# Fr4nz83/kubernetes-scheduler-simulator

Measured on AMD Instinct MI355X. Metric: pods scheduled/sec + node-score evals/sec (FGD, openb trace) at 1/2/4/8 MI355X, higher is better.
Workload: dtype int32+f64

## Files before the change

kubernetes-scheduler-simulator_amd/csrc/ksim_memo.hpp:

```cpp
#pragma once

namespace ksim_memo {

using namespace ksim;
using namespace ksim_plan::memo;

constexpr int kMBlock = 1024;
constexpr int kMWaves = kMBlock / 64;
constexpr int kMaxItems = 1 + 8 * kMaxCw;
constexpr int kCritWaves = 9;
constexpr unsigned kScanMask = 0x7C00u;
constexpr int kScanWaves = __builtin_popcount(kScanMask);
static_assert((kScanMask & ((2u << kCritWaves) - 1u)) == 0u && (kScanMask >> (kMWaves - 1)) == 0u,
              "the scan waves are idle in phase A on an owner too");
constexpr int kEvBuf = 128;
constexpr unsigned kSpinLimit = 1u << 22;
constexpr int kMaxDeadWords = 32;
constexpr int kLag = 3;
constexpr int kTopN = kLag + 1;
constexpr int kTopWords = 8;
constexpr int kDItems = kLag * 9;

struct MemoArgs {
  ReplicaDev* reps;
  const int* rep_list;
  const int* wg_map;
  int N, K, Cw;
  int nfw;
  int Cmax;
  const PodDev* cls_pod;
  const int* cls_owner;
  const int* wg_cls;
  const int* wg_ref;
  const unsigned long long* wg_grp;
  const int* ev_owner;
  const double* th;
  unsigned* win;
  int win_stride;
  int* fail;
  unsigned long long* prof;
  unsigned long long* trace;
  int trace_steps;
  int decider;
  const int* ev_cls;
  unsigned* topg;
  int skip;
  int delay;
  unsigned* hkeys;
  int* started;
  int gate_epoch;
};
constexpr int kTrace = 4;
constexpr int kProfPhases = 24;

struct __align__(16) MemoShared {
  PodDev ev[kEvBuf];
  int evo[kEvBuf + 8];
  unsigned dead[kMaxDeadWords];
  PodDev cls[kMaxCw];
  TypDev tp[kMaxTypical];
  NodeRec dnode;
  unsigned dfirst;
  unsigned pad_dfirst[3];
  double th[104];
  unsigned long long grp[kMaxCw];
  int cls_id[kMaxCw];
  int sc_ref[kMaxCw];
  int cnt[kMaxCw];
  unsigned ikey[kMaxItems + 3];
  double F[kMaxItems + 1];
  double Fc[10];
  uint8_t item_code[kMaxItems + 7];
  uint8_t item_slot[kMaxItems + 7];
  unsigned wtop[kMWaves][2];
  unsigned wtop4[kMWaves][kTopN];
  unsigned t2a, t2b;
  int nitems;
  int crit_done;
  int dirty;
  int stop;
  unsigned pay;
  unsigned long long prof[kProfPhases];
};
static_assert(sizeof(MemoShared) % 16 == 0, "keep the node records 16-B aligned");
static_assert(sizeof(MemoShared) == kSharedBytes, "memo_layout (ksim_plan.hpp) starts the node records after MemoShared");

KSIM_HD unsigned pack_key32(int score, int rank, int gf) {
  return ((unsigned)(score + 1) << 24) | ((unsigned)(kMemoMaxRank - rank) << 12) | ((unsigned)gf << 8);
}
KSIM_HD int key32_score(unsigned k) { return (int)(k >> 24) - 1; }
KSIM_HD int key32_rank(unsigned k) { return kMemoMaxRank - (int)((k >> 12) & 0xFFFu); }
KSIM_HD int key32_gpu(unsigned k) {
  const int gf = (int)((k >> 8) & 0xFu);
  return gf ? 15 - gf : -1;
}

KSIM_HD unsigned pack_pay(int rank, int mask) {
  return 1u | ((unsigned)(rank + 1) << 8) | ((unsigned)(mask & 0xff) << 24);
}

template <typename T>
__device__ __forceinline__ void gput(T* p, const T& v) {
  static_assert(sizeof(T) % 4 == 0, "word-sized records");
  const unsigned* src = reinterpret_cast<const unsigned*>(&v);
  __attribute__((address_space(1))) unsigned* dst = (__attribute__((address_space(1))) unsigned*)(p);
#pragma unroll
  for (int i = 0; i < (int)(sizeof(T) / 4); ++i) dst[i] = src[i];
}
template <typename T>
__device__ __forceinline__ T gget(const T* p) {
  static_assert(sizeof(T) % 4 == 0, "word-sized records");
  T v;
  unsigned* dst = reinterpret_cast<unsigned*>(&v);
  const __attribute__((address_space(1))) unsigned* src = (const __attribute__((address_space(1))) unsigned*)(p);
#pragma unroll
  for (int i = 0; i < (int)(sizeof(T) / 4); ++i) dst[i] = src[i];
  return v;
}
__device__ __forceinline__ void gput_node(NodeRec* p, const NodeV& n) {
  uint4* q = reinterpret_cast<uint4*>(p);
  gput(q, make_uint4((uint32_t)n.cpu_left, (uint32_t)n.mem_left, n.g[0], n.g[1]));
  gput(q + 1, make_uint4(n.g[2], n.g[3], n.meta, n.name_rank));
}

__device__ __forceinline__ unsigned gload32(const unsigned* p) {
  return __hip_atomic_load(p, __ATOMIC_RELAXED, __HIP_MEMORY_SCOPE_AGENT);
}
__device__ __forceinline__ void gstore32(unsigned* p, unsigned v) {
  __hip_atomic_store(p, v, __ATOMIC_RELAXED, __HIP_MEMORY_SCOPE_AGENT);
}
__device__ __forceinline__ double readlane_d(double v, int l) {
  const unsigned long long u = __builtin_bit_cast(unsigned long long, v);
  const unsigned lo = (unsigned)__builtin_amdgcn_readlane((int)(unsigned)u, l);
  const unsigned hi = (unsigned)__builtin_amdgcn_readlane((int)(unsigned)(u >> 32), l);
  return __builtin_bit_cast(double, ((unsigned long long)hi << 32) | lo);
}

__device__ __forceinline__ unsigned ge_mask(const NodeV& n, int m) {
  using ksim_replay::u16x2;
  const uint32_t mp = (uint32_t)m * 0x10001u;
  unsigned lt = 0u;
#pragma unroll
  for (int i = 0; i < 4; ++i) {
    const u16x2 d = (u16x2)(__builtin_bit_cast(u16x2, n.g[i]) - __builtin_bit_cast(u16x2, mp)) >> (u16x2){15, 15};
    const uint32_t x = __builtin_bit_cast(uint32_t, d);
    lt |= ((x & 1u) | ((x >> 15) & 2u)) << (2 * i);
  }
  return ~lt & 0xFFu;
}

__device__ __forceinline__ int score_lookup_dev(double delta, const double* th) {
  const float e = __builtin_amdgcn_exp2f((float)delta * -0.0014426950408889634f);
  int a = (int)(100.0f * __builtin_amdgcn_rcpf(1.0f + e));
  a = a < 0 ? 0 : (a > 100 ? 100 : a);
  if (delta >= th[a + 1]) ++a;
  else if (delta < th[a]) --a;
  return a;
}

__device__ __forceinline__ unsigned first_mask_lanes(const NodeV& n, int lane) {
  const int g = lane & 7;
  const int v = ksim_replay::gl_dyn(n, g);
  const bool first = lane < 8 && g < n.gpu_cnt() && (ksim_replay::gl_equal_mask(n, v) & ((1u << g) - 1u)) == 0u;
  return (unsigned)__ballot(first) & 0xFFu;
}

__device__ __forceinline__ void merge2(unsigned& a1, unsigned& a2, unsigned b1, unsigned b2) {
// ... 372 lines not shown
        if (lane == 0) s_last[rk] = step;
      }
      if (rk >= 0 && lane == 0) store_node(&ds.hprev[step % kLag], before);
      const unsigned fa = rk >= 0 ? first_mask_lanes(after, lane) : 0u;
      hn2 = hn1; ha2 = ha1; hf2 = hf1;
      hn1 = hn0; ha1 = ha0; hf1 = hf0;
      hn0 = rk; ha0 = after; hf0 = fa;
      dmark(23);
    }
    if (lane == 0) lds_store(&ds.finished, 1);
  } else if (wv == kPW) {
    int chunk = 0, my_cls = -1;
    for (int step = 0; step < E; ++step) {
      if (step == 0 || step - chunk >= 64) {
        chunk = step;
        my_cls = step + lane < E ? gget(a.ev_cls + gbase + step + lane) : -1;
      }
      if (__builtin_amdgcn_readlane(my_cls, step - chunk) < 0) continue;
      unsigned cspins = 0;
      while (lds_load(&ds.consumed) < step - kRing) {
        if (lds_load(&sh.stop) || lds_load(&ds.finished) || !lds_spin(cspins, &sh.stop, a.fail)) break;
      }
      if (lds_load(&sh.stop) || lds_load(&ds.finished)) break;
      unsigned v = 0u;
      bool ok = true;
      if (lane <= kTopN) {
        const unsigned* tw = a.topg + (gbase + step) * kTopWords;
        unsigned spins = 0;
        while ((v = gload32(tw + lane)) == 0u) {
          if (++spins > kSpinLimit || lds_load(&sh.stop)) { ok = false; break; }
          __builtin_amdgcn_s_sleep(1);
        }
      }
      if (__ballot(!ok) != 0ull) {
        if (lane == 0) { lds_store(&sh.stop, 1); atomicOr(a.fail, 1); }
        break;
      }
      const int slot = step % kRing;
      if (lane <= kTopN) ds.ring[slot][lane] = v;
      lds_release();
      if (lane == 0) lds_store(&ds.ring_tag[slot], step + 1);
    }
  } else if (wv <= nF) {
    int seen = 0;
    for (;;) {
      int cf;
      unsigned spins = 0;
      while ((cf = lds_load(&ds.cflag)) == seen) {
        if (lds_load(&ds.finished) || lds_load(&sh.stop) || !lds_spin(spins, &sh.stop, a.fail)) break;
        __builtin_amdgcn_s_sleep(2);
      }
      if (cf == seen) break;
      seen = cf;
      lds_acquire();
      const int nit = __builtin_amdgcn_readfirstlane(ds.nitems);
      const PodDev cp = ksim_replay::uniform_pod(&ds.cp);
      for (int it = wv - 1; it < nit; it += nF) {
        const NodeV cur = ksim_replay::uniform_node(&ds.xcur[ds.item_x[it]]);
        int cpuL, total;
        uint32_t gs[4];
        ksim_replay::fgd_candidate(cur, ds.item_code[it], cp, &cpuL, gs, &total);
        const double F = wave_F(cpuL, gs, total, 1u << cur.gpu_type(), rp.typed != 0, sh.tp, rp.ncpu, rp.nt, lane,
                                s_fold + (size_t)wv * kFoldBuf);
        if (lane == 0) ds.F[it] = F;
      }
      lds_release();
      if (lane == 0) __hip_atomic_fetch_add(&ds.fdone, 1, __ATOMIC_RELAXED, __HIP_MEMORY_SCOPE_WORKGROUP);
    }
  }
  __syncthreads();
}

template <bool kDecider, bool kGeneral, bool kStress = false, bool kReport = false, bool kHKeys = false>
__global__ __launch_bounds__(kMBlock) void k_memo(MemoArgs a, const TypDev* __restrict__ tp_all) {
  static_assert(!(kDecider && kHKeys), "the decider's scratch aliases the LDS keys");
  constexpr bool kDelays = kGeneral || kStress;
  extern __shared__ __attribute__((aligned(16))) char smem[];
  MemoShared& sh = *reinterpret_cast<MemoShared*>(smem);
  constexpr int kLW = kMWaves - 1;
  const int gw = a.wg_map[blockIdx.x];
  const int gi = gw >> 8;
  const int r = a.rep_list[gi];
  const int w = gw & 0xff;
  const int tid = (int)threadIdx.x, lane = tid & 63, wv = tid >> 6;
  const ReplicaDev rp = a.reps[r];
  const TypDev* __restrict__ tp = tp_all + (size_t)r * kMaxTypical;
  const int N = a.N, Cw = a.Cw;
  const int* rank2idx = reinterpret_cast<const int*>(rp.tags + (size_t)N * kTagStride);
  NodeRec* s_nodes = reinterpret_cast<NodeRec*>(smem + sizeof(MemoShared));
  unsigned* s_keys = kHKeys ? a.hkeys + (size_t)blockIdx.x * Cw * N : reinterpret_cast<unsigned*>(s_nodes + N);
  double* s_fold = reinterpret_cast<double*>(
      reinterpret_cast<char*>(s_nodes + N) + (kHKeys ? 0 : (std::max((size_t)Cw * N * 4, sizeof(DeciderScratch)) + 15) & ~(size_t)15));
  int* s_last = reinterpret_cast<int*>(reinterpret_cast<char*>(s_fold) +
                                       std::max((size_t)a.nfw * kFoldBuf * 8, ((size_t)N * 8 + 15) & ~(size_t)15));
  const PodDev* cls_pod = a.cls_pod + (size_t)gi * a.Cmax;
  const size_t wgo = (size_t)blockIdx.x * Cw;
  unsigned* win = a.win + (size_t)gi * a.win_stride;
  const int* evo = a.ev_owner + (size_t)gi * a.win_stride;
  const bool is_w0 = w == 0;
  constexpr bool kSkip = !kDecider && !kGeneral;
  const bool skip_ok = kSkip && a.skip && a.Cmax <= kMaxDeadWords * 32;

  for (int i = tid; i < N; i += kMBlock) {
    store_node(&s_nodes[i], load_node(rp.nodes + rank2idx[i]));
    s_last[i] = -1;
  }
  for (int j = tid; j < kMaxCw; j += kMBlock) {
    const int cid = j < Cw ? a.wg_cls[wgo + j] : -1;
    sh.cls_id[j] = cid;
    sh.sc_ref[j] = j < Cw ? a.wg_ref[wgo + j] : j;
    sh.grp[j] = j < Cw ? a.wg_grp[wgo + j] : 0ull;
    sh.cnt[j] = 0;
    if (cid >= 0) sh.cls[j] = cls_pod[cid];
    else reinterpret_cast<uint4*>(&sh.cls[j])[0] = reinterpret_cast<uint4*>(&sh.cls[j])[1] = make_uint4(0, 0, 0, 0);
  }
  for (int i = tid; i < rp.nt * 2; i += kMBlock)
    reinterpret_cast<uint4*>(sh.tp)[i] = reinterpret_cast<const uint4*>(tp)[i];
  if (tid == 0) { sh.dirty = -1; sh.stop = 0; sh.nitems = 0; sh.t2a = 0u; sh.t2b = 0u; sh.pay = 0u; sh.crit_done = 0; }
  if (a.started != nullptr && tid == 0)
    __hip_atomic_store(a.started + blockIdx.x, a.gate_epoch, __ATOMIC_RELAXED, __HIP_MEMORY_SCOPE_SYSTEM);
  for (int i = tid; i < kMaxDeadWords; i += kMBlock) sh.dead[i] = 0u;
  const bool prof = kGeneral && a.prof != nullptr;
  unsigned long long* const trace = kGeneral ? a.trace : nullptr;
  if (prof && tid < kProfPhases) sh.prof[tid] = 0ull;
  unsigned long long t_last = prof ? __builtin_amdgcn_s_memrealtime() : 0ull;
  const unsigned long long t_start = t_last, c_start = prof ? __builtin_amdgcn_s_memtime() : 0ull;
  auto mark = [&](int ph) {
    if (prof && tid == 0) {
      const unsigned long long t = __builtin_amdgcn_s_memrealtime();
      sh.prof[ph] += t - t_last;
      t_last = t;
    }
  };
  __syncthreads();
  double* s_F0 = s_fold;
  for (int i = tid; i < N; i += kMBlock) s_F0[i] = eval_fgd_item(load_node(&s_nodes[i]), 0, PodDev{}, rp, tp);
  __syncthreads();
  for (int x = tid; x < Cw * N; x += kMBlock) {
    const int j = x / N, i = x - j * N;
    unsigned k = 0u;
    if (sh.cls_id[j] >= 0) k = memo_key_scalar(load_node(&s_nodes[i]), sh.cls[j], s_F0[i], i, rp, tp);
    s_keys[x] = k;
  }
  __syncthreads();
  for (int i = tid; i < a.nfw * kFoldBuf; i += kMBlock) s_fold[i] = 0.0;
  for (int j = wv; j < Cw; j += kMWaves) {
    int c = 0;
    for (int i0 = 0; i0 < N; i0 += 64) c += __popcll(__ballot(i0 + lane < N && s_keys[(size_t)j * N + i0 + lane] != 0u));
    if (lane == 0) sh.cnt[j] = c;
  }

  auto top2 = [&](int slot) {
    const unsigned* kr = s_keys + (size_t)slot * N;
    unsigned a1 = 0u, a2 = 0u;
    for (int i = tid; i < N; i += kMBlock) {
      const unsigned k = kr[i];
      if (k > a1) { a2 = a1; a1 = k; } else if (k > a2) { a2 = k; }
    }
    wave_top2(a1, a2);
    if (lane == 0) { sh.wtop[wv][0] = a1; sh.wtop[wv][1] = a2; }
    __syncthreads();
    if (wv == 0) {
      a1 = lane < kMWaves ? sh.wtop[lane][0] : 0u;
      a2 = lane < kMWaves ? sh.wtop[lane][1] : 0u;
      wave_top2(a1, a2);
      if (lane == 0) { sh.t2a = a1; sh.t2b = a2; }
    }
  };
  const bool use_th = !kGeneral || a.th != nullptr;
  if (use_th)
    for (int i = tid; i < 102; i += kMBlock) sh.th[i] = a.th[i];
  const size_t gbase = (size_t)gi * a.win_stride;
  auto publish_top = [&](int slot, int sp) {
    const unsigned* kr = s_keys + (size_t)slot * N;
    unsigned k4[4];
#pragma unroll
    for (int q = 0; q < 4; ++q) k4[q] = tid + q * kMBlock < N ? kr[tid + q * kMBlock] : 0u;
    unsigned prev = 0xFFFFFFFFu;
#pragma unroll
    for (int r = 0; r < kTopN; ++r) {
      unsigned c = 0u;
#pragma unroll
      for (int q = 0; q < 4; ++q) c = (k4[q] < prev && k4[q] > c) ? k4[q] : c;
      const unsigned m = (unsigned)ksim_replay::wave_max_dpp((int)c);
      if (lane == 0) sh.wtop4[wv][r] = m;
      prev = m;
    }
    __syncthreads();
    if (wv == 0) {
      const unsigned v = lane < kMWaves * kTopN ? sh.wtop4[lane / kTopN][lane % kTopN] : 0u;
      unsigned pv = 0xFFFFFFFFu, out = 0u;
#pragma unroll
      for (int r = 0; r < kTopN; ++r) {
        const unsigned m = (unsigned)ksim_replay::wave_max_dpp((int)(v < pv ? v : 0u));
        out = lane == r ? m : out;
        pv = m;
      }
      unsigned* tw = a.topg + (gbase + sp) * kTopWords;
      if (lane < kTopN) gstore32(tw + lane, out | 1u);
      else if (lane == kTopN) gstore32(tw + lane, ((unsigned)sh.cnt[slot] << 8) | 1u);
    }
  };
  if constexpr (kDecider) {
    for (int sp = 0; sp < kLag && sp < rp.n_events; ++sp) {
      const int o = evo[sp];
      __syncthreads();
      if (o >= 0 && (o >> 16) == w) publish_top(o & 0xff, sp);
    }
  } else {
    int s0 = 0;
    while (s0 < rp.n_events && evo[s0] < 0) ++s0;
    __syncthreads();
    if (s0 < rp.n_events && (evo[s0] >> 16) == w) top2(evo[s0] & 0xff);
  }
  __syncthreads();
  mark(0);
  auto score_of = [&](double delta) { return use_th ? score_lookup_dev(delta, sh.th) : fgd_score_of_delta(delta); };

  PodDev lq{};
  bool l_valid = false, l_rep = false, l_share = false;
  int l_ref = 0;
  unsigned long long l_grp = 0ull;
  if (wv == kLW) {
    l_valid = lane < Cw && sh.cls_id[lane] >= 0;
    if (l_valid) lq = sh.cls[lane];
    l_ref = sh.sc_ref[lane];
    l_grp = sh.grp[lane];
    l_rep = l_valid && l_ref == lane;
    l_share = is_share_pod(lq);
  }
  bool r_feas = false, r_need = false, r_skip = false;
  int r_base = 0, r_ni = 0;

  const bool decider = kDecider && w == 0;
  if constexpr (kDecider)
    if (decider) memo_decider(a, rp, sh, s_nodes, *reinterpret_cast<DeciderScratch*>(s_keys), s_fold, s_last, gi, tid);
  for (int step = 0; step < (decider ? 0 : rp.n_events); ++step) {
    const int eb = step & (kEvBuf - 1);
    if (eb == 0) {
      const int ne = min(kEvBuf, rp.n_events - step);
      const uint4* src = reinterpret_cast<const uint4*>(rp.ev + step);
      for (int i = tid; i < ne * 2; i += kMBlock) reinterpret_cast<uint4*>(sh.ev)[i] = gget(src + i);
      for (int i = tid; i <= ne + kLag; i += kMBlock) sh.evo[i] = step + i < rp.n_events ? gget(evo + step + i) : -1;
      __syncthreads();
    }
    if constexpr (kSkip) {
      const int cls = __builtin_amdgcn_readfirstlane(sh.ev[eb].pad);
      if (skip_ok && ((sh.dead[cls >> 5] >> (cls & 31)) & 1u)) {
        const int wend = min(kEvBuf, rp.n_events - (step - eb));
        int run = wend - eb;
        for (int j0 = eb + 1; j0 < wend; j0 += 64) {
          const int j = j0 + lane;
          const int c = j < wend ? sh.ev[j].pad : 0;
          const unsigned long long lb = __ballot(j < wend && !((sh.dead[c >> 5] >> (c & 31)) & 1u));
          if (lb) {
            run = j0 + (int)__builtin_ctzll(lb) - eb;
            break;
          }
        }
        if (is_w0)
          for (int i = tid; i < run; i += kMBlock) gput(rp.res + step + i, ResultDev{-1, 0, 0, 0, ST_UNSCHED});
        if (step + run < rp.n_events) {
          const int ocn = __builtin_amdgcn_readfirstlane(sh.evo[eb + run]);
          if (ocn >= 0 && (ocn >> 16) == w) {
            __syncthreads();
            top2(ocn & 0xff);
          }
        }
        __syncthreads();
        step += run - 1;
        continue;
      }
    }
    if (trace && tid == 0 && step < a.trace_steps)
      trace[((size_t)blockIdx.x * a.trace_steps + step) * kTrace] = __builtin_amdgcn_s_memrealtime();
    if constexpr (kDelays) hdelay(a.delay, 4, step, wv, (int)blockIdx.x);
    const PodDev p = ksim_replay::uniform_pod(&sh.ev[eb]);
    const int oc = __builtin_amdgcn_readfirstlane(sh.evo[eb]);
    const int d = __builtin_amdgcn_readfirstlane(sh.dirty);
    const NodeV dn = ksim_replay::uniform_node(&sh.dnode);
    const unsigned dfirst = __builtin_amdgcn_readfirstlane(sh.dfirst);
    const bool del = kGeneral && (p.flags & kPodDelete) != 0u;
    const bool own = !kDecider && oc >= 0 && (oc >> 16) == w;
    const int oslot = own ? (oc & 0xff) : -1;
    const int crep = own ? ((oc >> 8) & 0xff) : -1;
    int nslot = -1;
    if constexpr (!kDecider) {
      if (step + 1 < rp.n_events) {
        const int ocn = __builtin_amdgcn_readfirstlane(sh.evo[eb + 1]);
        if (ocn >= 0 && (ocn >> 16) == w) {
          nslot = ocn & 0xff;
          if constexpr (kSkip) {
            const int cn = __builtin_amdgcn_readfirstlane(sh.cls_id[nslot]);
            if (skip_ok && ((sh.dead[cn >> 5] >> (cn & 31)) & 1u)) nslot = -1;
          }
        }
      }
    }
    const unsigned long long t_loaded = prof ? __builtin_amdgcn_s_memrealtime() : 0ull;
    if (prof && tid == 0) sh.prof[14] += t_loaded - t_last;

    if (d >= 0) {
      if (own && wv >= 1 && wv <= kCritWaves) {
        if constexpr (kDelays) hdelay(a.delay, 2, step, wv, (int)blockIdx.x);
        const PodDev cp = ksim_replay::uniform_pod(&sh.cls[crep]);
        const int c = wv - 1;
        int code = -1;
        if (c == 0) code = 0;
        else if (is_share_pod(cp)) code = (((dfirst & ge_mask(dn, cp.milli)) >> (c - 1)) & 1u) ? c : -1;
        else if (c == 1) code = 9;
        if (code >= 0) {
          int cpuL, total;
          uint32_t gs[4];
          ksim_replay::fgd_candidate(dn, code, cp, &cpuL, gs, &total);
          const double F = wave_F(cpuL, gs, total, 1u << dn.gpu_type(), rp.typed != 0, sh.tp, rp.ncpu, rp.nt, lane,
                                  s_fold + (size_t)wv * kFoldBuf);
          if (lane == 0) sh.Fc[c] = F;
        }
        if (lane == 0) {
          __builtin_amdgcn_fence(__ATOMIC_RELEASE, "workgroup");
          __hip_atomic_fetch_add(&sh.crit_done, 1, __ATOMIC_RELAXED, __HIP_MEMORY_SCOPE_WORKGROUP);
        }
      }
      if (wv == kLW) {
        const unsigned long long tl0 = prof ? __builtin_amdgcn_s_memrealtime() : 0ull;
        r_skip = own && l_valid && l_ref == crep;
        r_feas = l_valid && !r_skip && filter_node(dn, lq);
        const unsigned long long FM = __ballot(r_feas);
        r_need = l_rep && !r_skip && (FM & l_grp) != 0ull;
        unsigned cm = 0u;
        if (r_need) cm = l_share ? (dfirst & ge_mask(dn, lq.milli)) : 0x100u;
        r_ni = __popc(cm);
        int excl = 0, tot = 0;
#pragma unroll
        for (int b = 0; b < 4; ++b) {
          const unsigned long long m = __ballot((r_ni >> b) & 1);
          excl += __builtin_amdgcn_mbcnt_hi((unsigned)(m >> 32), __builtin_amdgcn_mbcnt_lo((unsigned)m, 0u)) << b;
          tot += __popcll(m) << b;
        }
        const int i0 = own ? 0 : 1;
        r_base = i0 + excl;
        int o = r_base;
        unsigned mm = cm;
        while (mm) {
          const int g = __builtin_ctz(mm);
          mm &= mm - 1u;
          sh.item_code[o] = (uint8_t)(l_share ? 1 + g : 9);
          sh.item_slot[o] = (uint8_t)lane;
          ++o;
        }
        if (lane == 0) {
          if (!own) {
            sh.item_code[0] = 0;
            sh.item_slot[0] = 0;
          }
          sh.nitems = tot > 0 ? i0 + tot : 0;
          if (prof) sh.prof[12] += __builtin_amdgcn_s_memrealtime() - tl0;
        }
      }
    }
    if constexpr (!kDecider) {
      if (nslot >= 0 && ((kScanMask >> wv) & 1u)) {
        const unsigned* kr = s_keys + (size_t)nslot * N;
        unsigned a1 = 0u, a2 = 0u;
        for (int i = __popc(kScanMask & ((1u << wv) - 1u)) * 64 + lane; i < N; i += kScanWaves * 64) {
          const unsigned k = i != d ? kr[i] : 0u;
          if (k > a1) { a2 = a1; a1 = k; } else if (k > a2) { a2 = k; }
        }
        wave_top2(a1, a2);
        if (lane == 0) { sh.wtop[wv][0] = a1; sh.wtop[wv][1] = a2; }
      }
    }
    unsigned gk_crit = 0u;
    if (own && wv == 0) {
      const unsigned t2a = sh.t2a, t2b = sh.t2b;
      const unsigned ex = (d >= 0 && t2a != 0u && key32_rank(t2a) == d) ? t2b : t2a;
      const bool ofeas = d >= 0 && filter_node(dn, ksim_replay::uniform_pod(&sh.cls[oslot]));
      const int mask_ex =
          ex != 0u ? select_gpus(load_node(&s_nodes[key32_rank(ex)]), p, rp.gpusel, key32_gpu(ex), rp.seed, step) : -1;
      const bool d_gpu_from_key = is_share_pod(p) && p.milli > 0 && (rp.gpusel == SEL_FGD || rp.gpusel == SEL_PWR);
      const bool early = d < 0 || !ofeas;
      int mask_d_pre = -1;
      unsigned W = 0u, pay = 0u;
      int rk = -1, mask = -1;
      auto publish = [&](unsigned fresh) {
        W = fresh > ex ? fresh : ex;
        rk = W != 0u ? key32_rank(W) : -1;
        const int gW = key32_gpu(W);
        mask = W == 0u ? -1 : (W == ex ? mask_ex : (d_gpu_from_key ? (gW < 0 ? -1 : 1 << gW) : mask_d_pre));
        pay = (W != 0u && mask >= 0) ? pack_pay(rk, mask) : (W == 0u ? 3u : 1u);
        if (lane == 0) {
          gstore32(win + step, pay);
          asm volatile("" ::: "memory");
          sh.pay = pay;
          if (prof) sh.prof[20] += __builtin_amdgcn_s_memrealtime() - t_loaded;
          if (trace && step < a.trace_steps)
            trace[((size_t)blockIdx.x * a.trace_steps + step) * kTrace + 1] = __builtin_amdgcn_s_memrealtime();
        }
      };
      if (early) publish(0u);
      const int cnt_o = sh.cnt[oslot];
      unsigned old_own = 0u, fresh = 0u;
      PodDev cp{};
      if (d >= 0) {
        old_own = s_keys[(size_t)oslot * N + d];
        cp = ksim_replay::uniform_pod(&sh.cls[crep]);
        if (ofeas && !d_gpu_from_key) mask_d_pre = select_gpus(dn, p, rp.gpusel, -1, rp.seed, step);
      }
      if (prof && tid == 0) sh.prof[16] += __builtin_amdgcn_s_memrealtime() - t_loaded;
      if (d >= 0) {
        if (lane == 0) {
          if constexpr (kDelays) {
            unsigned spins = 0;
            while (__hip_atomic_load(&sh.crit_done, __ATOMIC_RELAXED, __HIP_MEMORY_SCOPE_WORKGROUP) < kCritWaves) {
              if (++spins > 4 * kSpinLimit) {
                sh.stop = 1;
                atomicOr(a.fail, 32);
                break;
              }
              __builtin_amdgcn_s_sleep(0);
            }
          } else {
            while (__hip_atomic_load(&sh.crit_done, __ATOMIC_RELAXED, __HIP_MEMORY_SCOPE_WORKGROUP) < kCritWaves)
              __builtin_amdgcn_s_sleep(0);
          }
          sh.crit_done = 0;
          if (prof) sh.prof[17] += __builtin_amdgcn_s_memrealtime() - t_loaded;
          if (trace && step < a.trace_steps)
            trace[((size_t)blockIdx.x * a.trace_steps + step) * kTrace + 3] = __builtin_amdgcn_s_memrealtime();
        }
        __builtin_amdgcn_fence(__ATOMIC_ACQUIRE, "workgroup");
        __builtin_amdgcn_wave_barrier();
        const bool cshare = is_share_pod(cp);
        const unsigned fm = cshare ? (dfirst & ge_mask(dn, cp.milli)) : 0u;
        const bool has = lane >= 1 && lane <= 8 && (cshare ? ((fm >> (lane - 1)) & 1u) != 0u : lane == 1);
        int k = 0;
        if (has) k = (int)pack_key32(score_of(sh.Fc[0] - sh.Fc[lane]), d, cshare ? 15 - (lane - 1) : 0);
        const unsigned gk = (unsigned)ksim_replay::wave_max_dpp(k);
        const unsigned z = pack_key32(0, d, 0);
        gk_crit = gk > z ? gk : z;
        fresh = ofeas ? gk_crit : 0u;
        if (prof && tid == 0) sh.prof[18] += __builtin_amdgcn_s_memrealtime() - t_loaded;
        if (trace && lane == 0 && step < a.trace_steps)
          trace[((size_t)blockIdx.x * a.trace_steps + step) * kTrace + 2] = __builtin_amdgcn_s_memrealtime();
      }
      if (!early) publish(fresh);
      if (lane == 0) {
        const int nfeas = cnt_o + (d >= 0 ? (fresh != 0u ? 1 : 0) - (old_own != 0u ? 1 : 0) : 0);
        ResultDev out{-1, 0, 0, nfeas, ST_UNSCHED};
        if (W != 0u) {
          if (mask < 0) {
            out.status = ST_ERROR;
          } else {
            out.status = ST_OK;
            out.score = result_score(rp, nfeas, key32_score(W), 0, 0);
            out.node = rk;
            out.gpu_mask = mask;
          }
        }
        gput(rp.res + step, out);
        if (prof) sh.prof[19] += __builtin_amdgcn_s_memrealtime() - t_loaded;
      }
      if (d >= 0) {
        const int j = lane;
        if (j < Cw && ((sh.grp[crep] >> j) & 1ull)) {
          const PodDev q = sh.cls[j];
          const unsigned nk = filter_node(dn, q) ? gk_crit : 0u;
          unsigned* kp = s_keys + (size_t)j * N + d;
          const unsigned old = *kp;
          *kp = nk;
          sh.cnt[j] += (nk != 0u ? 1 : 0) - (old != 0u ? 1 : 0);
        }
      }
    }
    if (prof && tid == 0 && own) sh.prof[15] += __builtin_amdgcn_s_memrealtime() - t_loaded;
    mark(1);
    __syncthreads();
    mark(2);
    mark(3);
    if (d >= 0) {
      const int nit = __builtin_amdgcn_readfirstlane(sh.nitems);
      if (wv < a.nfw) {
        double* fb = s_fold + (size_t)wv * kFoldBuf;
        for (int it = wv; it < nit; it += a.nfw) {
          const int code = sh.item_code[it];
          const PodDev q = ksim_replay::uniform_pod(&sh.cls[sh.item_slot[it]]);
          int cpuL, total;
          uint32_t gs[4];
          ksim_replay::fgd_candidate(dn, code, q, &cpuL, gs, &total);
          const double F = wave_F(cpuL, gs, total, 1u << dn.gpu_type(), rp.typed != 0, sh.tp, rp.ncpu, rp.nt, lane, fb);
          if (lane == 0) sh.F[it] = F;
        }
      }
    }
    mark(4);
    __syncthreads();
    mark(5);
    unsigned nk_l = 0u;
    if (d >= 0 && wv == kLW) {
      const unsigned long long tl0 = prof ? __builtin_amdgcn_s_memrealtime() : 0ull;
      const int nit = __builtin_amdgcn_readfirstlane(sh.nitems);
      const double F0 = own ? sh.Fc[0] : sh.F[0];
      for (int it = (own ? 0 : 1) + lane; it < nit; it += 64) {
        const int code = sh.item_code[it];
        sh.ikey[it] = pack_key32(score_of(F0 - sh.F[it]), d, code <= 8 ? 15 - (code - 1) : 0);
      }
      __builtin_amdgcn_fence(__ATOMIC_RELEASE, "wavefront");
      __builtin_amdgcn_wave_barrier();
      unsigned gk = r_need ? pack_key32(0, d, 0) : 0u;
      for (int k = 0; k < r_ni; ++k) {
        const unsigned x = sh.ikey[r_base + k];
        gk = x > gk ? x : gk;
      }
      const unsigned gkj = __shfl(gk, l_valid ? l_ref : 0, 64);
      if (l_valid && !r_skip) {
        const unsigned nk = r_feas ? gkj : 0u;
        unsigned* kp = s_keys + (size_t)lane * N + d;
        const unsigned old = *kp;
        *kp = nk;
        nk_l = nk;
        sh.cnt[lane] += (nk != 0u ? 1 : 0) - (old != 0u ? 1 : 0);
      }
      if (prof && lane == 0) sh.prof[13] += __builtin_amdgcn_s_memrealtime() - tl0;
    }
    mark(6);
    if constexpr (kDecider) {
      if (step + kLag < rp.n_events) {
        const int ocn = __builtin_amdgcn_readfirstlane(sh.evo[eb + kLag]);
        if (ocn >= 0 && (ocn >> 16) == w) {
          __syncthreads();
          publish_top(ocn & 0xff, step + kLag);
        }
      }
    } else if (nslot >= 0 && wv == kLW) {
      int sw = -1;
#pragma unroll
      for (int k = 0, m = (int)kScanMask; k < kScanWaves; ++k, m &= m - 1) sw = lane == k ? __builtin_ctz(m) : sw;
      unsigned a1 = sw >= 0 ? sh.wtop[sw][0] : 0u, a2 = sw >= 0 ? sh.wtop[sw][1] : 0u;
      wave_top2(a1, a2);
      if (d >= 0) {
        const bool own_grp = ((__ballot(r_skip) >> nslot) & 1ull) != 0ull;
        const unsigned fk = own_grp ? s_keys[(size_t)nslot * N + d] : (unsigned)__builtin_amdgcn_readlane((int)nk_l, nslot);
        merge2(a1, a2, fk, 0u);
      }
      if (lane == 0) { sh.t2a = a1; sh.t2b = a2; }
    }
    mark(7);
    if constexpr (kDelays) hdelay(a.delay, 1, step, wv, (int)blockIdx.x);
    if (wv == 0) {
      int nd_w = -1;
      NodeV nn{};
      if (lane == 0) {
      unsigned pay = 0u;
      int sign = +1;
      PodDev bp = p;
      bool ok = true;
      if (del) {
        sign = -1;
        if (p.ref >= 0 && p.ref < step) {
          pay = gload32(win + p.ref);
          bp = gget(rp.ev + p.ref);
        }
      } else if (own) {
        pay = sh.pay;
      } else {
        unsigned spins = 0;
        while ((pay = gload32(win + step)) == 0u) {
          if (++spins > kSpinLimit) { ok = false; break; }
          __builtin_amdgcn_s_sleep(1);
        }
        if (trace && step < a.trace_steps)
          trace[((size_t)blockIdx.x * a.trace_steps + step) * kTrace + 1] = __builtin_amdgcn_s_memrealtime();
      }
      int nd = -1;
      if (kSkip && skip_ok && ok && (pay & 2u))
        sh.dead[p.pad >> 5] |= 1u << (p.pad & 31);
      if (!ok) {
        sh.stop = 1;
        atomicOr(a.fail, 1);
      } else {
        const int rk = (int)((pay >> 8) & 0xffffu) - 1;
        const int mask = (int)(pay >> 24);
        if (rk >= 0) {
          NodeV n = load_node(&s_nodes[rk]);
          bind_node(n, bp, mask, sign);
          store_node(&s_nodes[rk], n);
          store_node(&sh.dnode, n);
          nn = n;
          if (del && is_w0) gput(rp.res + step, ResultDev{rk, mask, 0, 0, ST_DELETED});
          if ((kGeneral || kReport) && rp.snap && (del ? is_w0 : own)) {
            gput_node(rp.snap + step, n);
            gput(rp.prev + step, s_last[rk]);
          }
          s_last[rk] = step;
          nd = rk;
        } else if (del && is_w0) {
          gput(rp.res + step, ResultDev{-1, 0, 0, 0, ST_DELETED});
        }
      }
      sh.dirty = nd;
      nd_w = nd;
      }
      nd_w = __builtin_amdgcn_readfirstlane(nd_w);
      if (nd_w >= 0) {
        NodeV u;
        u.cpu_left = __builtin_amdgcn_readfirstlane(nn.cpu_left);
        u.mem_left = __builtin_amdgcn_readfirstlane(nn.mem_left);
#pragma unroll
        for (int i = 0; i < 4; ++i) u.g[i] = __builtin_amdgcn_readfirstlane(nn.g[i]);
        u.meta = __builtin_amdgcn_readfirstlane(nn.meta);
        u.name_rank = __builtin_amdgcn_readfirstlane(nn.name_rank);
        const unsigned fmk = first_mask_lanes(u, lane);
        if (lane == 0) sh.dfirst = fmk;
      }
    }
    mark(8);
    __syncthreads();
    mark(9);
    if (sh.stop) break;
  }
  if (prof && tid == 0) {
    sh.prof[10] = __builtin_amdgcn_s_memtime() - c_start;
    sh.prof[11] = __builtin_amdgcn_s_memrealtime() - t_start;
  }
  __syncthreads();
  if (prof && tid < kProfPhases) a.prof[(size_t)blockIdx.x * kProfPhases + tid] = sh.prof[tid];
  if (is_w0 && !sh.stop)
    for (int i = tid; i < N; i += kMBlock) store_node(rp.nodes + rank2idx[i], load_node(&s_nodes[i]));
}

__global__ void k_memo_finish(ReplicaDev* reps, const int* rep_list, int N) {
  const ReplicaDev rp = reps[rep_list[blockIdx.y]];
  const int e = (int)(blockIdx.x * blockDim.x + threadIdx.x);
  if (e >= rp.n_events) return;
  const int* rank2idx = reinterpret_cast<const int*>(rp.tags + (size_t)N * kTagStride);
  ResultDev r = rp.res[e];
  if (r.node < 0) return;
  const int idx = rank2idx[r.node];
  rp.res[e].node = idx;
  const PodDev p = rp.ev[e];
  const bool del = (p.flags & kPodDelete) != 0u;
  if (!(del ? r.status == ST_DELETED : r.status == ST_OK)) return;
  const int tag = del ? rp.ev[p.ref].tag : p.tag;
  if (tag < 0) return;
  const size_t h = (size_t)idx * kTagStride + tag;
  unsigned* word = reinterpret_cast<unsigned*>(rp.tags) + (h >> 1);
  atomicAdd(word, (unsigned)(del ? -1 : 1) << (16 * (h & 1)));
}

}
```

kubernetes-scheduler-simulator_amd/csrc/ksim_replay.hpp:

```cpp
#pragma once

namespace ksim_replay {

using namespace ksim;
using ksim_plan::replay::kMaxK;
using ksim_plan::replay::kPfGuess;
using ksim_plan::replay::RLayout;
using ksim_plan::replay::replay_layout;

constexpr int kRBlock = 1024;
constexpr int kRWaves = kRBlock / 64;
constexpr int kChunk = kRBlock;
constexpr int kFChunk = kRBlock / 8;
constexpr int kRMaxCand = 9;
constexpr int kGran = 3;
constexpr int kGranW = 10;
constexpr unsigned kSpinLimit = 1u << 22;
constexpr int kEvBuf = 128;

struct ReplayArgs {
  ReplicaDev* reps;
  const int* rep_list;
  int N;
  int K;
// ... 60 lines not shown
__device__ __forceinline__ unsigned long long gload(const unsigned long long* p) {
  return __hip_atomic_load(p, __ATOMIC_RELAXED, __HIP_MEMORY_SCOPE_AGENT);
}
__device__ __forceinline__ void gstore(unsigned long long* p, unsigned long long v) {
  __hip_atomic_store(p, v, __ATOMIC_RELAXED, __HIP_MEMORY_SCOPE_AGENT);
}

template <int kCtrl>
__device__ __forceinline__ int dpp_i(int v) {
  return __builtin_amdgcn_update_dpp(0, v, kCtrl, 0xF, 0xF, false);
}
template <int kCtrl>
__device__ __forceinline__ unsigned long long dpp_u64(unsigned long long v) {
  const int lo = dpp_i<kCtrl>((int)(unsigned)v), hi = dpp_i<kCtrl>((int)(unsigned)(v >> 32));
  return ((unsigned long long)(unsigned)hi << 32) | (unsigned)lo;
}
__device__ __forceinline__ unsigned long long readlane_u64(unsigned long long v, int l) {
  const unsigned lo = (unsigned)__builtin_amdgcn_readlane((int)(unsigned)v, l);
  const unsigned hi = (unsigned)__builtin_amdgcn_readlane((int)(unsigned)(v >> 32), l);
  return ((unsigned long long)hi << 32) | lo;
}
__device__ __forceinline__ unsigned long long wave_max_u64_dpp(unsigned long long v) {
  unsigned long long w;
  w = dpp_u64<0xB1>(v); v = w > v ? w : v;
  w = dpp_u64<0x4E>(v); v = w > v ? w : v;
  w = dpp_u64<0x141>(v); v = w > v ? w : v;
  w = dpp_u64<0x140>(v); v = w > v ? w : v;
  const unsigned long long a = readlane_u64(v, 0), b = readlane_u64(v, 16), c = readlane_u64(v, 32),
                           d = readlane_u64(v, 48);
  const unsigned long long x = a > b ? a : b, y = c > d ? c : d;
  return x > y ? x : y;
}
__device__ __forceinline__ int wave_sum_dpp(int v) {
  v += dpp_i<0xB1>(v);
  v += dpp_i<0x4E>(v);
  v += dpp_i<0x141>(v);
  v += dpp_i<0x140>(v);
  return __builtin_amdgcn_readlane(v, 0) + __builtin_amdgcn_readlane(v, 16) + __builtin_amdgcn_readlane(v, 32) +
         __builtin_amdgcn_readlane(v, 48);
}
__device__ __forceinline__ int wave_min_dpp(int v) {
  v = min(v, dpp_i<0xB1>(v));
  v = min(v, dpp_i<0x4E>(v));
  v = min(v, dpp_i<0x141>(v));
  v = min(v, dpp_i<0x140>(v));
  return min(min(__builtin_amdgcn_readlane(v, 0), __builtin_amdgcn_readlane(v, 16)),
             min(__builtin_amdgcn_readlane(v, 32), __builtin_amdgcn_readlane(v, 48)));
}
__device__ __forceinline__ int wave_max_dpp(int v) {
  v = max(v, dpp_i<0xB1>(v));
  v = max(v, dpp_i<0x4E>(v));
  v = max(v, dpp_i<0x141>(v));
  v = max(v, dpp_i<0x140>(v));
  return max(max(__builtin_amdgcn_readlane(v, 0), __builtin_amdgcn_readlane(v, 16)),
             max(__builtin_amdgcn_readlane(v, 32), __builtin_amdgcn_readlane(v, 48)));
}

__device__ __forceinline__ int group8_max(int v) {
  v = max(v, dpp_i<0xB1>(v));
  v = max(v, dpp_i<0x4E>(v));
  v = max(v, dpp_i<0x141>(v));
  return v;
}

__device__ __forceinline__ int gl_dyn(const NodeV& n, int g) {
  const uint32_t w01 = (g & 2) ? n.g[1] : n.g[0];
  const uint32_t w23 = (g & 2) ? n.g[3] : n.g[2];
  const uint32_t w = (g & 4) ? w23 : w01;
  return (int)((g & 1) ? (w >> 16) : (w & 0xffffu));
}

__device__ __forceinline__ unsigned gl_equal_mask(const NodeV& n, int v) {
  const uint32_t vv = (uint32_t)v * 0x10001u;
  unsigned m = 0u;
#pragma unroll
  for (int i = 0; i < 4; ++i) {
    const uint32_t x = n.g[i] ^ vv;
    m |= ((x & 0xffffu) == 0u ? 1u : 0u) << (2 * i);
    m |= ((x >> 16) == 0u ? 1u : 0u) << (2 * i + 1);
  }
  return m;
}

__device__ __forceinline__ PodDev uniform_pod(const PodDev* s) {
  const uint4* q = reinterpret_cast<const uint4*>(s);
  uint4 x = q[0], y = q[1];
  x.x = __builtin_amdgcn_readfirstlane(x.x); x.y = __builtin_amdgcn_readfirstlane(x.y);
  x.z = __builtin_amdgcn_readfirstlane(x.z); x.w = __builtin_amdgcn_readfirstlane(x.w);
  y.x = __builtin_amdgcn_readfirstlane(y.x); y.y = __builtin_amdgcn_readfirstlane(y.y);
  y.z = __builtin_amdgcn_readfirstlane(y.z); y.w = __builtin_amdgcn_readfirstlane(y.w);
  PodDev p;
  uint4* o = reinterpret_cast<uint4*>(&p);
  o[0] = x;
  o[1] = y;
  return p;
}

__device__ __forceinline__ NodeV uniform_node(const NodeRec* s) {
  NodeV n = load_node(s);
  n.cpu_left = __builtin_amdgcn_readfirstlane(n.cpu_left);
  n.mem_left = __builtin_amdgcn_readfirstlane(n.mem_left);
#pragma unroll
  for (int i = 0; i < 4; ++i) n.g[i] = __builtin_amdgcn_readfirstlane(n.g[i]);
  n.meta = __builtin_amdgcn_readfirstlane(n.meta);
  n.name_rank = __builtin_amdgcn_readfirstlane(n.name_rank);
  return n;
}

template <int J>
__device__ __forceinline__ int qbc(int v) {
  return __builtin_amdgcn_mov_dpp(v, J * 0x55, 0xF, 0xF, true);
}
template <int J>
__device__ __forceinline__ double qbc_d(double v) {
  const unsigned long long u = __builtin_bit_cast(unsigned long long, v);
  const unsigned lo = (unsigned)qbc<J>((int)(unsigned)u), hi = (unsigned)qbc<J>((int)(unsigned)(u >> 32));
  return __builtin_bit_cast(double, ((unsigned long long)hi << 32) | lo);
}

typedef unsigned short u16x2 __attribute__((ext_vector_type(2)));

__device__ __forceinline__ double sel01(bool f) {
  return __builtin_bit_cast(double, (unsigned long long)(f ? 0x3FF00000u : 0u) << 32);
}

__device__ __forceinline__ void fgd_candidate(const NodeV& m, int code, const PodDev& p, int* cpuL,
                                              uint32_t (&g)[4], int* total) {
  *cpuL = m.cpu_left;
#pragma unroll
  for (int i = 0; i < 4; ++i) g[i] = m.g[i];
  unsigned mask = 0u;
  if (code >= 1 && code <= 8) {
    mask = 1u << (code - 1);
  } else if (code == 9) {
    int gl[kMaxGpu];
    unpack_gl(m, gl);
    bool ok = false;
    mask = sub_gpu_mask(gl, m.gpu_cnt(), *cpuL, p, &ok);
    if (!ok) mask = 0u;
    if (ok) *cpuL -= p.cpu_nz;
  }
  if (code >= 1 && code <= 8) *cpuL -= p.cpu_nz;
  const uint32_t d = (uint32_t)(uint16_t)p.milli;
#pragma unroll
  for (int i = 0; i < 4; ++i)
    g[i] -= (((mask >> (2 * i)) & 1u) ? d : 0u) + (((mask >> (2 * i + 1)) & 1u) ? (d << 16) : 0u);
  uint32_t t = 0u;
#pragma unroll
  for (int i = 0; i < 4; ++i) t = __builtin_amdgcn_udot2(__builtin_bit_cast(u16x2, g[i]), (u16x2){1, 1}, t, false);
  *total = (int)t;
}

template <bool kTyped>
__device__ __forceinline__ double frag_F_quad(int cpuL, const uint32_t (&g)[4], int total, uint32_t typebit,
                                              const TypDev* __restrict__ tp, const TypDev* ltp, int ncpu, int nt,
                                              int q) {
  (void)tp;
  const double dtot = (double)total;
  double bc = 0.0;
  for (int tb = 0; tb < ncpu; tb += 4) {
    const int t = min(tb + q, max(nt - 1, 0));
    const double x = ltp[t].freq * dtot;
    int code = cpuL >= ltp[t].cpu ? 0 : 1;
    code = tb + q < ncpu ? code : 4;
    int cj;
    double vj;
    cj = qbc<0>(code); vj = qbc_d<0>(x); bc = __builtin_fma(vj, sel01(cj == q), bc);
    cj = qbc<1>(code); vj = qbc_d<1>(x); bc = __builtin_fma(vj, sel01(cj == q), bc);
    cj = qbc<2>(code); vj = qbc_d<2>(x); bc = __builtin_fma(vj, sel01(cj == q), bc);
    cj = qbc<3>(code); vj = qbc_d<3>(x); bc = __builtin_fma(vj, sel01(cj == q), bc);
  }
  double bg = 0.0;
  const int tmax = max(nt - 1, 0);
  for (int tb0 = ncpu; tb0 < nt; tb0 += 8) {
    const TypDev e2[2] = {ltp[min(tb0 + q, tmax)], ltp[min(tb0 + 4 + q, tmax)]};
#pragma unroll
    for (int h = 0; h < 2; ++h) {
      const int tb = tb0 + 4 * h;
      const TypDev e = e2[h];
      const uint32_t mp = (uint32_t)e.milli * 0x10001u;
      uint32_t frag = 0u, nlt = 0u;
#pragma unroll
      for (int i = 0; i < 4; ++i) {
        const u16x2 gv = __builtin_bit_cast(u16x2, g[i]);
        const u16x2 lt = (u16x2)(gv - __builtin_bit_cast(u16x2, mp)) >> (u16x2){15, 15};
        frag = __builtin_amdgcn_udot2(gv, lt, frag, false);
        nlt = __builtin_amdgcn_udot2(lt, (u16x2){1, 1}, nlt, false);
      }
      const bool gpu_ok = kMaxGpu - (int)nlt >= e.num_eff;
      const bool cpu_ok = cpuL >= e.cpu;
// ... 128 lines not shown
```

Measured before the change: 3.700 million.

## Prefetch next event's static LDS data and batch step-start shared loads

Reorders MemoShared so dirty/stop sit next to dfirst, which lets each step read dfirst, dirty and stop with one 16-byte LDS load and t2a/t2b with one 8-byte load. The next event's pod, owner codes and dead-class bits are prefetched into registers after the mid-step barrier, replacing the serialized LDS reads and readfirstlane chains at step start. The class pod is now taken from the event pod instead of being re-read from sh.cls, and the stop check moves to the top of the loop. This shortens LDS latency on the per-event critical path at the cost of more live registers and extra layout invariants.

Result: slower. 3.547 million (-4.1%).

```diff
diff --git a/kubernetes-scheduler-simulator_amd/csrc/ksim_memo.hpp b/kubernetes-scheduler-simulator_amd/csrc/ksim_memo.hpp
--- a/kubernetes-scheduler-simulator_amd/csrc/ksim_memo.hpp
+++ b/kubernetes-scheduler-simulator_amd/csrc/ksim_memo.hpp
@@ -61,7 +61,9 @@
   TypDev tp[kMaxTypical];
   NodeRec dnode;
   unsigned dfirst;
-  unsigned pad_dfirst[3];
+  int dirty;
+  int stop;
+  unsigned pad_stop;
   double th[104];
   unsigned long long grp[kMaxCw];
   int cls_id[kMaxCw];
@@ -77,12 +79,14 @@
   unsigned t2a, t2b;
   int nitems;
   int crit_done;
-  int dirty;
-  int stop;
   unsigned pay;
+  unsigned pad_pay[2];
   unsigned long long prof[kProfPhases];
 };
 static_assert(sizeof(MemoShared) % 16 == 0, "keep the node records 16-B aligned");
+static_assert(offsetof(MemoShared, dnode) % 16 == 0 && offsetof(MemoShared, dfirst) == offsetof(MemoShared, dnode) + 32 &&
+                  offsetof(MemoShared, t2a) % 8 == 0,
+              "the step start reads dnode | dfirst, dirty, stop | t2a, t2b with 16-B and 8-B loads");
 static_assert(sizeof(MemoShared) == kSharedBytes, "memo_layout (ksim_plan.hpp) starts the node records after MemoShared");
 
 KSIM_HD unsigned pack_key32(int score, int rank, int gf) {
@@ -621,7 +625,7 @@
   const int gi = gw >> 8;
   const int r = a.rep_list[gi];
   const int w = gw & 0xff;
-  const int tid = (int)threadIdx.x, lane = tid & 63, wv = tid >> 6;
+  const int tid = (int)threadIdx.x, lane = tid & 63, wv = __builtin_amdgcn_readfirstlane(tid >> 6);
   const ReplicaDev rp = a.reps[r];
   const TypDev* __restrict__ tp = tp_all + (size_t)r * kMaxTypical;
   const int N = a.N, Cw = a.Cw;
@@ -774,6 +778,33 @@
   const bool decider = kDecider && w == 0;
   if constexpr (kDecider)
     if (decider) memo_decider(a, rp, sh, s_nodes, *reinterpret_cast<DeciderScratch*>(s_keys), s_fold, s_last, gi, tid);
+  constexpr bool kPre = !kDecider;
+  uint4 pf_x = make_uint4(0, 0, 0, 0), pf_y = pf_x;
+  int pf_oc = -1, pf_ocn = -1, pf_cn = 0;
+  bool pf = false;
+  auto load_static = [&](int e) {
+    const uint4* q = reinterpret_cast<const uint4*>(&sh.ev[e]);
+    pf_x = q[0];
+    pf_y = q[1];
+    pf_oc = sh.evo[e];
+    if constexpr (!kDecider) {
+      pf_ocn = sh.evo[e + 1];
+      if constexpr (kSkip) pf_cn = sh.ev[min(e + 1, kEvBuf - 1)].pad;
+    }
+  };
+  auto pf_uniform = [&]() {
+    pf_x.x = __builtin_amdgcn_readfirstlane(pf_x.x); pf_x.y = __builtin_amdgcn_readfirstlane(pf_x.y);
+    pf_x.z = __builtin_amdgcn_readfirstlane(pf_x.z); pf_x.w = __builtin_amdgcn_readfirstlane(pf_x.w);
+    pf_y.x = __builtin_amdgcn_readfirstlane(pf_y.x); pf_y.y = __builtin_amdgcn_readfirstlane(pf_y.y);
+    pf_y.z = __builtin_amdgcn_readfirstlane(pf_y.z); pf_y.w = __builtin_amdgcn_readfirstlane(pf_y.w);
+    pf_oc = __builtin_amdgcn_readfirstlane(pf_oc);
+    pf_ocn = __builtin_amdgcn_readfirstlane(pf_ocn);
+    pf_cn = __builtin_amdgcn_readfirstlane(pf_cn);
+  };
+  auto prefetch = [&](int e) {
+    pf = e < kEvBuf;
+    if (pf) load_static(e);
+  };
   for (int step = 0; step < (decider ? 0 : rp.n_events); ++step) {
     const int eb = step & (kEvBuf - 1);
     if (eb == 0) {
@@ -783,9 +814,28 @@
       for (int i = tid; i <= ne + kLag; i += kMBlock) sh.evo[i] = step + i < rp.n_events ? gget(evo + step + i) : -1;
       __syncthreads();
     }
+    if (!pf) load_static(eb);
+    pf = false;
+    uint4 hd = *reinterpret_cast<const uint4*>(&sh.dfirst);
+    NodeV dn = load_node(&sh.dnode);
+    uint2 t2 = *reinterpret_cast<const uint2*>(&sh.t2a);
+    unsigned dwc = 0u, dwn = 0u;
     if constexpr (kSkip) {
-      const int cls = __builtin_amdgcn_readfirstlane(sh.ev[eb].pad);
-      if (skip_ok && ((sh.dead[cls >> 5] >> (cls & 31)) & 1u)) {
+      dwc = sh.dead[((int)pf_y.w >> 5) & (kMaxDeadWords - 1)];
+      dwn = sh.dead[(pf_cn >> 5) & (kMaxDeadWords - 1)];
+    }
+    pf_uniform();
+    asm volatile("" : "+v"(hd.x), "+v"(hd.y), "+v"(hd.z), "+v"(t2.x), "+v"(t2.y), "+v"(dwc), "+v"(dwn), "+v"(dn.cpu_left),
+                      "+v"(dn.mem_left), "+v"(dn.g[0]), "+v"(dn.g[1]), "+v"(dn.g[2]), "+v"(dn.g[3]), "+v"(dn.meta),
+                      "+v"(dn.name_rank));
+    PodDev p;
+    reinterpret_cast<uint4*>(&p)[0] = pf_x;
+    reinterpret_cast<uint4*>(&p)[1] = pf_y;
+    const int oc = pf_oc, ocn = pf_ocn;
+    if (__builtin_amdgcn_readfirstlane(hd.z)) break;
+    if constexpr (kSkip) {
+      const int cls = p.pad;
+      if (skip_ok && ((__builtin_amdgcn_readfirstlane(dwc) >> (cls & 31)) & 1u)) {
         const int wend = min(kEvBuf, rp.n_events - (step - eb));
         int run = wend - eb;
         for (int j0 = eb + 1; j0 < wend; j0 += 64) {
@@ -800,12 +850,13 @@
         if (is_w0)
           for (int i = tid; i < run; i += kMBlock) gput(rp.res + step + i, ResultDev{-1, 0, 0, 0, ST_UNSCHED});
         if (step + run < rp.n_events) {
-          const int ocn = __builtin_amdgcn_readfirstlane(sh.evo[eb + run]);
-          if (ocn >= 0 && (ocn >> 16) == w) {
+          const int ocr = __builtin_amdgcn_readfirstlane(sh.evo[eb + run]);
+          if (ocr >= 0 && (ocr >> 16) == w) {
             __syncthreads();
-            top2(ocn & 0xff);
+            top2(ocr & 0xff);
           }
         }
+        if constexpr (kPre) prefetch(eb + run);
         __syncthreads();
         step += run - 1;
         continue;
@@ -814,25 +865,24 @@
     if (trace && tid == 0 && step < a.trace_steps)
       trace[((size_t)blockIdx.x * a.trace_steps + step) * kTrace] = __builtin_amdgcn_s_memrealtime();
     if constexpr (kDelays) hdelay(a.delay, 4, step, wv, (int)blockIdx.x);
-    const PodDev p = ksim_replay::uniform_pod(&sh.ev[eb]);
-    const int oc = __builtin_amdgcn_readfirstlane(sh.evo[eb]);
-    const int d = __builtin_amdgcn_readfirstlane(sh.dirty);
-    const NodeV dn = ksim_replay::uniform_node(&sh.dnode);
-    const unsigned dfirst = __builtin_amdgcn_readfirstlane(sh.dfirst);
+    const int d = __builtin_amdgcn_readfirstlane(hd.y);
+    dn = ksim_replay::uniform_node(dn);
+    const unsigned dfirst = __builtin_amdgcn_readfirstlane(hd.x);
     const bool del = kGeneral && (p.flags & kPodDelete) != 0u;
     const bool own = !kDecider && oc >= 0 && (oc >> 16) == w;
     const int oslot = own ? (oc & 0xff) : -1;
     const int crep = own ? ((oc >> 8) & 0xff) : -1;
     int nslot = -1;
     if constexpr (!kDecider) {
-      if (step + 1 < rp.n_events) {
-        const int ocn = __builtin_amdgcn_readfirstlane(sh.evo[eb + 1]);
-        if (ocn >= 0 && (ocn >> 16) == w) {
-          nslot = ocn & 0xff;
-          if constexpr (kSkip) {
-            const int cn = __builtin_amdgcn_readfirstlane(sh.cls_id[nslot]);
-            if (skip_ok && ((sh.dead[cn >> 5] >> (cn & 31)) & 1u)) nslot = -1;
+      if (step + 1 < rp.n_events && ocn >= 0 && (ocn >> 16) == w) {
+        nslot = ocn & 0xff;
+        if constexpr (kSkip) {
+          int cn = pf_cn;
+          if (eb + 1 >= kEvBuf) {
+            cn = __builtin_amdgcn_readfirstlane(sh.cls_id[nslot]);
+            dwn = sh.dead[cn >> 5];
           }
+          if (skip_ok && ((__builtin_amdgcn_readfirstlane(dwn) >> (cn & 31)) & 1u)) nslot = -1;
         }
       }
     }
@@ -842,7 +892,7 @@
     if (d >= 0) {
       if (own && wv >= 1 && wv <= kCritWaves) {
         if constexpr (kDelays) hdelay(a.delay, 2, step, wv, (int)blockIdx.x);
-        const PodDev cp = ksim_replay::uniform_pod(&sh.cls[crep]);
+        const PodDev& cp = p;
         const int c = wv - 1;
         int code = -1;
         if (c == 0) code = 0;
@@ -912,9 +962,9 @@
     }
     unsigned gk_crit = 0u;
     if (own && wv == 0) {
-      const unsigned t2a = sh.t2a, t2b = sh.t2b;
+      const unsigned t2a = t2.x, t2b = t2.y;
       const unsigned ex = (d >= 0 && t2a != 0u && key32_rank(t2a) == d) ? t2b : t2a;
-      const bool ofeas = d >= 0 && filter_node(dn, ksim_replay::uniform_pod(&sh.cls[oslot]));
+      const bool ofeas = d >= 0 && filter_node(dn, p);
       const int mask_ex =
           ex != 0u ? select_gpus(load_node(&s_nodes[key32_rank(ex)]), p, rp.gpusel, key32_gpu(ex), rp.seed, step) : -1;
       const bool d_gpu_from_key = is_share_pod(p) && p.milli > 0 && (rp.gpusel == SEL_FGD || rp.gpusel == SEL_PWR);
@@ -943,7 +993,7 @@
       PodDev cp{};
       if (d >= 0) {
         old_own = s_keys[(size_t)oslot * N + d];
-        cp = ksim_replay::uniform_pod(&sh.cls[crep]);
+        cp = p;
         if (ofeas && !d_gpu_from_key) mask_d_pre = select_gpus(dn, p, rp.gpusel, -1, rp.seed, step);
       }
       if (prof && tid == 0) sh.prof[16] += __builtin_amdgcn_s_memrealtime() - t_loaded;
@@ -1035,6 +1085,7 @@
     mark(4);
     __syncthreads();
     mark(5);
+    if constexpr (kPre) prefetch(eb + 1);
     unsigned nk_l = 0u;
     if (d >= 0 && wv == kLW) {
       const unsigned long long tl0 = prof ? __builtin_amdgcn_s_memrealtime() : 0ull;
@@ -1156,7 +1207,6 @@
     mark(8);
     __syncthreads();
     mark(9);
-    if (sh.stop) break;
   }
   if (prof && tid == 0) {
     sh.prof[10] = __builtin_amdgcn_s_memtime() - c_start;
diff --git a/kubernetes-scheduler-simulator_amd/csrc/ksim_replay.hpp b/kubernetes-scheduler-simulator_amd/csrc/ksim_replay.hpp
--- a/kubernetes-scheduler-simulator_amd/csrc/ksim_replay.hpp
+++ b/kubernetes-scheduler-simulator_amd/csrc/ksim_replay.hpp
@@ -166,9 +166,7 @@
   return m;
 }
 
-__device__ __forceinline__ PodDev uniform_pod(const PodDev* s) {
-  const uint4* q = reinterpret_cast<const uint4*>(s);
-  uint4 x = q[0], y = q[1];
+__device__ __forceinline__ PodDev uniform_pod(uint4 x, uint4 y) {
   x.x = __builtin_amdgcn_readfirstlane(x.x); x.y = __builtin_amdgcn_readfirstlane(x.y);
   x.z = __builtin_amdgcn_readfirstlane(x.z); x.w = __builtin_amdgcn_readfirstlane(x.w);
   y.x = __builtin_amdgcn_readfirstlane(y.x); y.y = __builtin_amdgcn_readfirstlane(y.y);
@@ -179,9 +177,12 @@
   o[1] = y;
   return p;
 }
-
-__device__ __forceinline__ NodeV uniform_node(const NodeRec* s) {
-  NodeV n = load_node(s);
+__device__ __forceinline__ PodDev uniform_pod(const PodDev* s) {
+  const uint4* q = reinterpret_cast<const uint4*>(s);
+  return uniform_pod(q[0], q[1]);
+}
+
+__device__ __forceinline__ NodeV uniform_node(NodeV n) {
   n.cpu_left = __builtin_amdgcn_readfirstlane(n.cpu_left);
   n.mem_left = __builtin_amdgcn_readfirstlane(n.mem_left);
 #pragma unroll
@@ -190,6 +191,7 @@
   n.name_rank = __builtin_amdgcn_readfirstlane(n.name_rank);
   return n;
 }
+__device__ __forceinline__ NodeV uniform_node(const NodeRec* s) { return uniform_node(load_node(s)); }
 
 template <int J>
 __device__ __forceinline__ int qbc(int v) {
```
